# wolfbox/snappy

Hardware: AMD Instinct MI355X
Metric: GiB/s hashed (whole node), bit-exact hashes.yaml, 10k x 1 MiB tree (higher is better)
Workload: dtype u64; 1 GPU; C2: ONE on-disk tree (tmpfs) of 10001 files (10 000 x 1 MiB + the 1 MiB archive stand-in) -> hashes.yaml, sharded over 1 rank(s) on 1 distinct GPU(s); bytes=10486808576, kernel=sha512_split_kernel<true>, tree_home=/dev/shm

## Files before the change

snappy_amd/csrc/hostfill.cpp:

```cpp
#include "hostfill.h"

#include <new>

#include <ctype.h>
#include <dirent.h>
#include <errno.h>
#include <sched.h>
#include <stdio.h>
#include <string.h>
#include <sys/syscall.h>
#include <unistd.h>

#include <algorithm>
#include <atomic>

#if defined(__x86_64__)
#include <immintrin.h>
#endif

namespace snaphash {

namespace {

bool read_small_file(const std::string& path, std::string& out)
{
    FILE* f = fopen(path.c_str(), "r");
    if (!f) return false;
    char buf[4096];
    out.clear();
    size_t r;
    while ((r = fread(buf, 1, sizeof buf, f)) > 0) out.append(buf, r);
    fclose(f);
    return true;
}

constexpr int kMpolDefault = 0, kMpolPreferred = 1;
constexpr unsigned kMpolFNode = 1u << 0, kMpolFAddr = 1u << 1;

}

std::vector<int> parse_cpulist(const std::string& text)
{
    std::vector<int> out;
    const char* p = text.c_str();
    while (*p) {
        while (*p && !isdigit((unsigned char)*p)) ++p;
        if (!*p) break;
        char* end = nullptr;
        const long a = strtol(p, &end, 10);
        long b = a;
        p = end;
        if (*p == '-') { b = strtol(p + 1, &end, 10); p = end; }
        if (a < 0 || b < a || b - a > 65536) break;
        for (long c = a; c <= b; ++c) out.push_back((int)c);
    }
    return out;
}

int numa_node_of_pci(const std::string& sysfs_root, const std::string& bdf_in)
{
    std::string bdf = bdf_in;
    for (char& c : bdf) c = (char)tolower((unsigned char)c);
    if (bdf.empty()) return -1;
    std::string text;
    if (!read_small_file(sysfs_root + "/bus/pci/devices/" + bdf + "/numa_node", text)) return -1;
    char* end = nullptr;
    const long v = strtol(text.c_str(), &end, 10);
    if (end == text.c_str()) return -1;
    return v < 0 ? -1 : (int)v;
}

std::vector<int> numa_cpus_of_node(const std::string& sysfs_root, int node)
{
    std::string text;
    if (node < 0 || !read_small_file(sysfs_root + "/devices/system/node/node" + std::to_string(node) + "/cpulist", text)) return {};
    return parse_cpulist(text);
}

std::vector<int> slice_cpus(const std::vector<int>& all, size_t pos, size_t m)
{
    if (m < 2 || pos >= m) return all;
    std::vector<int> mine;
    for (size_t a = 0; a < all.size();) {
        size_t b = a + 1;
        while (b < all.size() && all[b] == all[b - 1] + 1) ++b;
        const size_t len = b - a;
        for (size_t i = a + len * pos / m; i < a + len * (pos + 1) / m; ++i) mine.push_back(all[i]);
        a = b;
    }
    return mine;
}

int numa_node_count(const std::string& sysfs_root)
{
    int n = 0;
    if (DIR* d = opendir((sysfs_root + "/devices/system/node").c_str())) {
        while (struct dirent* de = readdir(d))
            if (!strncmp(de->d_name, "node", 4) && isdigit((unsigned char)de->d_name[4])) ++n;
        closedir(d);
    }
    return n;
}

bool numa_prefer_node(int node, SavedMemPolicy* saved)
{
#if defined(SYS_set_mempolicy) && defined(SYS_get_mempolicy)
    if (node < 0 || node >= 1024) return false;
    saved->valid = syscall(SYS_get_mempolicy, &saved->mode, saved->mask, (unsigned long)1024 + 1, nullptr, 0ul) == 0;
    unsigned long mask[1024 / (8 * sizeof(unsigned long))] = {0};
    mask[(size_t)node / (8 * sizeof(unsigned long))] |= 1ul << ((size_t)node % (8 * sizeof(unsigned long)));
    return syscall(SYS_set_mempolicy, kMpolPreferred, mask, (unsigned long)1024 + 1) == 0;
#else
    (void)node; (void)saved;
    return false;
#endif
}

void numa_restore_policy(const SavedMemPolicy& saved)
{
#if defined(SYS_set_mempolicy)
    if (saved.valid && saved.mode != kMpolDefault &&
        syscall(SYS_set_mempolicy, saved.mode, saved.mask, (unsigned long)1024 + 1) == 0)
        return;
    (void)syscall(SYS_set_mempolicy, kMpolDefault, nullptr, 0ul);
#else
    (void)saved;
#endif
}

int numa_node_of_address(const void* addr)
{
#if defined(SYS_get_mempolicy)
    int node = -1;
    if (syscall(SYS_get_mempolicy, &node, nullptr, 0ul, addr, (unsigned long)(kMpolFNode | kMpolFAddr)) != 0) return -1;
    return node;
#else
    (void)addr;
    return -1;
#endif
}

unsigned cgroup_cpu_quota(const std::string& sysfs_cgroup_root, const std::string& proc_self_cgroup)
{
    std::string text;
    if (!read_small_file(proc_self_cgroup, text)) return 0;
    double best = 0;
    auto take = [&](double quota, double period) {
        if (quota > 0 && period > 0) { const double c = quota / period; if (best == 0 || c < best) best = c; }
    };
    size_t pos = 0;
    while (pos < text.size()) {
        size_t eol = text.find('\n', pos);
        if (eol == std::string::npos) eol = text.size();
        const std::string line = text.substr(pos, eol - pos);
        pos = eol + 1;
        const size_t c1 = line.find(':'), c2 = c1 == std::string::npos ? c1 : line.find(':', c1 + 1);
        if (c2 == std::string::npos) continue;
        const std::string ctrl = line.substr(c1 + 1, c2 - c1 - 1);
        std::string path = line.substr(c2 + 1);
        const bool v2 = ctrl.empty();
        if (!v2) {
            bool has_cpu = false;
            for (size_t a = 0; a <= ctrl.size();) {
                size_t b = ctrl.find(',', a);
                if (b == std::string::npos) b = ctrl.size();
                if (ctrl.compare(a, b - a, "cpu") == 0) has_cpu = true;
                a = b + 1;
            }
            if (!has_cpu) continue;
        }
        const std::string base = sysfs_cgroup_root + (v2 ? "" : "/" + ctrl);
        for (;;) {
            std::string v;
            if (v2) {
                if (read_small_file(base + path + "/cpu.max", v) && v.compare(0, 3, "max") != 0) {
                    char* end = nullptr;
                    const double q = strtod(v.c_str(), &end);
                    const double per = end ? strtod(end, nullptr) : 0;
                    take(q, per);
                }
            } else {
                std::string pv;
                if (read_small_file(base + path + "/cpu.cfs_quota_us", v) && read_small_file(base + path + "/cpu.cfs_period_us", pv))
                    take(strtod(v.c_str(), nullptr), strtod(pv.c_str(), nullptr));
            }
            if (path.empty() || path == "/") break;
            const size_t slash = path.rfind('/');
            path = slash == 0 || slash == std::string::npos ? "/" : path.substr(0, slash);
        }
    }
    if (best <= 0) return 0;
    return (unsigned)std::max(1.0, best + 0.5);
}

unsigned usable_cpus()
{
    unsigned n = 0;
    cpu_set_t set;
    CPU_ZERO(&set);
    if (sched_getaffinity(0, sizeof set, &set) == 0) {
        const int c = CPU_COUNT(&set);
        if (c > 0) n = (unsigned)c;
    }
    if (n == 0) n = std::max(1u, std::thread::hardware_concurrency());
    static const unsigned quota = cgroup_cpu_quota("/sys/fs/cgroup", "/proc/self/cgroup");
    if (quota && quota < n) n = quota;
    return n;
}


FillPool::~FillPool() { stop(); }

void FillPool::stop()
{
    {
        std::lock_guard<std::mutex> lk(mu_);
        quit_ = true;
    }
    cv_work_.notify_all();
    for (auto& t : th_) if (t.joinable()) t.join();
    th_.clear();
    quit_ = false;
}

void FillPool::configure(unsigned max_threads, const std::vector<int>& cpus)
{
    stop();
    max_threads_ = max_threads;
    cpus_ = cpus;
}

void FillPool::worker(unsigned id)
{
    if (!cpus_.empty()) {
        cpu_set_t set, allowed;
        CPU_ZERO(&set);
        CPU_ZERO(&allowed);
        const bool have_allowed = sched_getaffinity(0, sizeof allowed, &allowed) == 0;
        for (int c : cpus_)
            if (c >= 0 && c < CPU_SETSIZE && (!have_allowed || CPU_ISSET(c, &allowed))) CPU_SET(c, &set);
        if (CPU_COUNT(&set) > 0) (void)sched_setaffinity(0, sizeof set, &set);
    }
    uint64_t seen = 0;
    for (;;) {
        const std::function<void(size_t)>* fn;
        size_t n;
        std::atomic<size_t>* next;
        {
            std::unique_lock<std::mutex> lk(mu_);
            cv_work_.wait(lk, [&] { return quit_ || (epoch_ != seen && id < want_); });
            if (quit_) return;
            seen = epoch_;
            fn = fn_; n = n_; next = next_;
        }
        try {
            for (;;) {
                const size_t i = next->fetch_add(1);
                if (i >= n) break;
                (*fn)(i);
            }
        } catch (...) {
            fn_threw_.store(true);
        }
        {
            std::lock_guard<std::mutex> lk(mu_);
            if (--running_ == 0) cv_done_.notify_all();
        }
    }
}

void FillPool::parallel_for(size_t n, unsigned threads, const std::function<void(size_t)>& fn)
{
    if (n == 0) return;
    unsigned helpers = threads > 1 ? std::min(threads - 1, max_threads_) : 0u;
    if (helpers > n - 1) helpers = (unsigned)(n - 1);
    std::atomic<size_t> next{0};
    if (helpers) {
        std::lock_guard<std::mutex> lk(mu_);
        try {
            while (th_.size() < helpers) { const unsigned id = (unsigned)th_.size(); th_.emplace_back(&FillPool::worker, this, id); }
        } catch (...) {
            helpers = (unsigned)th_.size();
        }
        if (helpers) {
            fn_ = &fn; n_ = n; next_ = &next;
            want_ = helpers;
            running_ = helpers;
            ++epoch_;
        }
    }
    if (helpers) cv_work_.notify_all();
    bool threw = false;
    try {
        for (;;) {
            const size_t i = next.fetch_add(1);
            if (i >= n) break;
            fn(i);
        }
    } catch (...) {
        threw = true;
        next.store(n);
    }
    if (helpers) {
        std::unique_lock<std::mutex> lk(mu_);
        cv_done_.wait(lk, [&] { return running_ == 0; });
        want_ = 0;
        fn_ = nullptr; next_ = nullptr;
    }
    if (fn_threw_.exchange(false) || threw) throw std::bad_alloc();
}


void run_on_threads(unsigned T, const std::function<void(unsigned)>& fn)
{
    if (T <= 1) { fn(0); return; }
    static std::mutex mu;
    static FillPool* pool = [] {
        FillPool* p = new FillPool();
        p->configure(64, {});
        return p;
    }();
    static const pid_t born_in = getpid();
    if (T <= 65 && getpid() == born_in && mu.try_lock()) {
        std::lock_guard<std::mutex> lk(mu, std::adopt_lock);
        pool->parallel_for(T, T, [&fn](size_t t) { fn((unsigned)t); });
        return;
    }
    ThreadJoiner th;
    for (unsigned t = 1; t < T; ++t) th.spawn(fn, t);
    fn(0);
    th.join_all();
}


#if defined(__x86_64__)
namespace {
__attribute__((target("avx2"))) void copy_nt_avx2(uint8_t* dst, const uint8_t* src, size_t n)
{
    const size_t head = (64 - ((uintptr_t)dst & 63)) & 63;
    if (head) { memcpy(dst, src, head); dst += head; src += head; n -= head; }
    size_t lines = n / 64;
    while (lines--) {
        const __m256i a = _mm256_loadu_si256((const __m256i*)src);
        const __m256i b = _mm256_loadu_si256((const __m256i*)(src + 32));
        _mm256_stream_si256((__m256i*)dst, a);
        _mm256_stream_si256((__m256i*)(dst + 32), b);
        src += 64; dst += 64;
    }
    n &= 63;
    if (n) memcpy(dst, src, n);
    _mm_sfence();
}
const bool g_have_avx2 = __builtin_cpu_supports("avx2");
}
#endif

void copy_to_staging(void* dst, const void* src, size_t n)
{
#if defined(__x86_64__)
    if (n >= (32u << 10) && g_have_avx2) { copy_nt_avx2((uint8_t*)dst, (const uint8_t*)src, n); return; }
#endif
    memcpy(dst, src, n);
}

}
```

snappy_amd/csrc/hostfill.h:

```cpp
#pragma once
#include <stddef.h>
#include <stdint.h>

#include <atomic>
#include <condition_variable>
#include <functional>
#include <mutex>
#include <new>
#include <string>
#include <thread>
#include <vector>

namespace snaphash {

int numa_node_of_pci(const std::string& sysfs_root, const std::string& bdf);
std::vector<int> numa_cpus_of_node(const std::string& sysfs_root, int node);
std::vector<int> parse_cpulist(const std::string& text);
int numa_node_count(const std::string& sysfs_root);
std::vector<int> slice_cpus(const std::vector<int>& all, size_t pos, size_t m);

struct SavedMemPolicy {
    bool valid = false;
    int mode = 0;
    unsigned long mask[1024 / (8 * sizeof(unsigned long)) + 1] = {0};
};
bool numa_prefer_node(int node, SavedMemPolicy* saved);
void numa_restore_policy(const SavedMemPolicy& saved);
int numa_node_of_address(const void* addr);
unsigned usable_cpus();
unsigned cgroup_cpu_quota(const std::string& sysfs_cgroup_root, const std::string& proc_self_cgroup);

struct ThreadJoiner {
    std::vector<std::thread> th;
    std::atomic<bool> worker_threw{false};
    ThreadJoiner() = default;
    ThreadJoiner(const ThreadJoiner&) = delete;
    ThreadJoiner& operator=(const ThreadJoiner&) = delete;
    ~ThreadJoiner() { join_quietly(); }
    template <class F, class... A> void spawn(F&& f, A&&... a)
    {
        th.emplace_back([this](auto fn, auto... args) {
            try { fn(args...); } catch (...) { worker_threw.store(true); }
        }, std::forward<F>(f), std::forward<A>(a)...);
    }
    void join_quietly()
    {
        for (auto& t : th)
            if (t.joinable()) t.join();
    }
    void join_all()
    {
        join_quietly();
        if (worker_threw.exchange(false)) throw std::bad_alloc();
    }
};

class FillPool {
public:
    FillPool() = default;
    ~FillPool();
    FillPool(const FillPool&) = delete;
    FillPool& operator=(const FillPool&) = delete;
    void configure(unsigned max_threads, const std::vector<int>& cpus);
    void parallel_for(size_t n, unsigned threads, const std::function<void(size_t)>& fn);
    unsigned max_threads() const { return max_threads_; }
    const std::vector<int>& cpus() const { return cpus_; }

private:
    void worker(unsigned id);
    void stop();
    unsigned max_threads_ = 0;
    std::vector<int> cpus_;
    std::vector<std::thread> th_;
    std::mutex mu_;
    std::condition_variable cv_work_, cv_done_;
    uint64_t epoch_ = 0;
    unsigned want_ = 0;
    unsigned running_ = 0;
    bool quit_ = false;
    const std::function<void(size_t)>* fn_ = nullptr;
    std::atomic<bool> fn_threw_{false};
    size_t n_ = 0;
    std::atomic<size_t>* next_ = nullptr;
};

void run_on_threads(unsigned T, const std::function<void(unsigned)>& fn);

void copy_to_staging(void* dst, const void* src, size_t n);

}
```

snappy_amd/csrc/snaphash_api.cpp:

```cpp
#include <dirent.h>
#include <errno.h>
#include <fcntl.h>
#include <hip/hip_runtime.h>
#include <string.h>
#include <sys/resource.h>
#include <sys/stat.h>
#include <time.h>
#include <unistd.h>

#include <algorithm>
#include <atomic>
#include <queue>
#include <chrono>
#include <string>
#include <thread>
#include <unordered_map>
#include <vector>

#include <dlfcn.h>
#include <rccl/rccl.h>

#include <condition_variable>
#include <functional>
#include <future>
#include <memory>
#include <mutex>

#include "batchplan.h"
#include "engine_bufs.h"
#include "gpu_handles.h"
#include "hostfill.h"
#include "hostpass.h"
#include "hostsha.h"
#include "inflate_host.h"
#include "member_hashers.h"
#include "planner.h"
#include "sha512_core.h"
#include "sha512_kernels.h"
#include "snap_core.h"
#include "tarpack.h"
#include "walk.h"

using namespace snaphash;

namespace {

constexpr uint64_t kDefaultStaging = 256ull << 20;

double now_ms()
{
    using namespace std::chrono;
    return duration<double, std::milli>(steady_clock::now().time_since_epoch()).count();
}

}

struct snaphash_ctx;

struct DevCtx {
    int device = 0;
    int index = 0;
    Stream stream;
    Stream copy_stream;
    uint64_t staging = kDefaultStaging;
    uint32_t kernel_pref = SNAPHASH_KERNEL_AUTO;
    uint32_t deflate_depth = 0;
    uint32_t n_xcd = 8;

    std::vector<SubSlot> sub;
    Slot slot[3];
    HashBufs hash;
    Twin<CmpChunk> cmp;
    DeflateBufs z;
    Stream z_stream;
    Stream z2_stream;
    std::vector<Event> z_ev;
    std::vector<Event> z_part_ev;
    InflateBufs inf;
    Bzip2Bufs bz;
    CrcBufs crc;
    Sha256Bufs sha256;
    BcjBufs bcj;
    Event bcj_ev[2];
    hipStream_t bcj_busy = nullptr;
    XzBufs xz;
    XzEncBufs xe;
    BzEncBufs be;
    Stream f_stream;
    uint64_t fout_gen = 0;

    EventLedger ledger;
    bool pending = false;

    std::string pci_bus_id;
    int numa_node = -1;
    int staging_node = -1;
    int64_t fd_budget = 0;
    int64_t fd_call_budget = -1;
    unsigned fill_cap = 12;
    unsigned fill_call_cap = 0;
    snaphash_ctx* owner = nullptr;
    unsigned owner_cpus_per_engine = 0;
    uint64_t staged_calls = 0;
    double fill_thread_s = 0;
    uint64_t fill_bytes = 0;
    FillPool pool;

    snaphash_stats stats{};
    double t_call0 = 0;
    std::string last_error;

    template <class F> void each_buf(F&& f)
    {
        for (Slot& s : slot) s.each(f);
        for (SubSlot& q : sub) q.jobs.each(f);
        hash.each(f);
        cmp.each(f);
        z.each(f);
        inf.each(f);
        bz.each(f);
        crc.each(f);
        sha256.each(f);
        bcj.each(f);
        xz.each(f);
        xe.each(f);
        be.each(f);
    }
};

namespace {
struct Rccl {
    void* lib = nullptr;
    bool tried = false, ok = false;
    std::string why;
    ncclResult_t (*CommInitAll)(ncclComm_t*, int, const int*) = nullptr;
    ncclResult_t (*CommDestroy)(ncclComm_t) = nullptr;
    ncclResult_t (*AllGather)(const void*, void*, size_t, ncclDataType_t, ncclComm_t, hipStream_t) = nullptr;
    ncclResult_t (*GroupStart)() = nullptr;
    ncclResult_t (*GroupEnd)() = nullptr;
    const char* (*GetErrorString)(ncclResult_t) = nullptr;
    std::vector<ncclComm_t> comms;
};
}

struct snaphash_batch;

struct snaphash_ctx {
    std::vector<std::unique_ptr<DevCtx>> dev;
    uint32_t host_threads = 0;
    bool gpu_only = false;
    unsigned cpus = 1;
    unsigned cpus_call = 0;
    double host_rate = 1.4e9;
    PlanCalib calib;
    std::mutex calib_mu;
    uint32_t flags = 0;
    Rccl rccl;
    std::vector<DevBuf<uint8_t>> d_gather;
    snaphash_stats stats{};
    snaphash_stats_ex ex{};
    snaphash_targz_stats targz{};
    snaphash_unpack_stats unpack{};
    snaphash_xz_check_stats xz_check{};
    snaphash_xz_selfcheck_stats xz_selfcheck{};
    snaphash_xz_filter_stats xz_filter{};
    bool unxz_bcj = false;
    snaphash_bz2_selfcheck_stats bz2_selfcheck{};
    snaphash_block_scan_stats block_scan{};
    std::string last_error;
    snaphash_batch* open_batch = nullptr;
    DevCtx* d0() const { return dev[0].get(); }
};

namespace {

int fail(DevCtx* c, int code, const std::string& msg)
{
    if (c) c->last_error = msg;
    return code;
}
int fail(snaphash_ctx* x, int code, const std::string& msg)
{
// ... 81 lines not shown
    else (void)hipHostFree(p);
}

namespace {

int ensure_slots(DevCtx* c, int nslots = 2, uint64_t want = 0)
{
    if (want == 0 || want > c->staging) want = c->staging;
    for (int k = 0; k < nslots; ++k) {
        Slot& s = c->slot[k];
        HIP_TRY(c, s.ensure(want, c->numa_node));
        if (c->staging_node < 0) { s.h_buf[0] = 0; c->staging_node = numa_node_of_address(s.h_buf.data()); }
        HIP_TRY(c, s.done.ensure(hipEventDisableTiming));
        HIP_TRY(c, s.copied.ensure(hipEventDisableTiming));
    }
    HIP_TRY(c, c->copy_stream.ensure(hipStreamNonBlocking));
    return SNAPHASH_OK;
}

constexpr size_t kSplitMaxStreams = 32768;
constexpr uint64_t kSplitMinBlocks = 32;

uint64_t job_blocks(const Job& j) { return (j.nbytes >> 7) + 1; }

hipError_t launch_kernel(uint32_t k, const Job* d_jobs, size_t n, DevCtx* c, uint8_t* d_digests, bool staged)
{
    if (k == SNAPHASH_KERNEL_QUAD) return launch_quad(d_jobs, (uint32_t)n, c->hash.d_state.data(), d_digests, c->stream);
    if (k == SNAPHASH_KERNEL_PAIR) return launch_pair(d_jobs, (uint32_t)n, c->hash.d_state.data(), d_digests, c->stream, staged);
    if (k == SNAPHASH_KERNEL_SPLIT) return launch_split(d_jobs, (uint32_t)n, c->hash.d_state.data(), d_digests, c->stream);
    return launch_wide(d_jobs, (uint32_t)n, c->hash.d_state.data(), d_digests, c->stream);
}

size_t plan_kernels(const DevCtx* c, const Job* h_jobs, size_t n, uint32_t* k_head, uint32_t* k_tail)
{
    *k_tail = SNAPHASH_KERNEL_WIDE;
    if (c->kernel_pref == SNAPHASH_KERNEL_WIDE || c->kernel_pref == SNAPHASH_KERNEL_SPLIT ||
        c->kernel_pref == SNAPHASH_KERNEL_PAIR || c->kernel_pref == SNAPHASH_KERNEL_QUAD) {
        *k_head = c->kernel_pref;
        return n;
    }
    *k_head = SNAPHASH_KERNEL_PAIR;
    uint64_t blocks = 0;
    for (size_t i = 0; i < n; ++i) blocks += job_blocks(h_jobs[i]);
    if (n <= kSplitMaxStreams) {
        if (blocks >= kSplitMinBlocks * n) return n;
        *k_head = SNAPHASH_KERNEL_WIDE;
        return n;
    }
    if (job_blocks(h_jobs[0]) >= 8 * job_blocks(h_jobs[kSplitMaxStreams - 1]) &&
        job_blocks(h_jobs[0]) >= kSplitMinBlocks) {
        size_t head = 0;
        while (head < kSplitMaxStreams && job_blocks(h_jobs[head]) >= kSplitMinBlocks) ++head;
        return head;
    }
    *k_head = SNAPHASH_KERNEL_WIDE;
    return n;
}

int launch_jobs(DevCtx* c, Job* h_jobs, Job* d_jobs, size_t n, uint8_t* d_digests, hipEvent_t copied = nullptr)
{
    if (n == 0) return SNAPHASH_OK;
    std::stable_sort(h_jobs, h_jobs + n, [](const Job& a, const Job& b) { return a.nbytes > b.nbytes; });
    if (copied) {
        HIP_TRY(c, hipMemcpyAsync(d_jobs, h_jobs, n * sizeof(Job), hipMemcpyHostToDevice, c->copy_stream));
        HIP_TRY(c, hipEventRecord(copied, c->copy_stream));
        HIP_TRY(c, hipStreamWaitEvent(c->stream, copied, 0));
    } else {
        HIP_TRY(c, hipMemcpyAsync(d_jobs, h_jobs, n * sizeof(Job), hipMemcpyHostToDevice, c->stream));
    }
    uint32_t k_head, k_tail;
    const size_t head = plan_kernels(c, h_jobs, n, &k_head, &k_tail);
    Span ev;
    if (int rc = span_begin(c, Ev::Hash, c->stream, &ev)) return rc;
    const bool staged = copied != nullptr;
    hipError_t e = launch_kernel(k_head, d_jobs, head, c, d_digests, staged);
    if (e == hipSuccess && head < n) e = launch_kernel(k_tail, d_jobs + head, n - head, c, d_digests, staged);
    if (e != hipSuccess) return fail(c, SNAPHASH_EDEVICE, std::string("kernel launch: ") + hipGetErrorString(e));
    if (int rc = span_end(c, ev, c->stream)) return rc;
    c->stats.launches += (head < n) ? 2 : 1;
    c->stats.kernel_used = k_head;
    c->pending = true;
    return SNAPHASH_OK;
}

int sync_ctx(DevCtx* c)
{
    if (!c->pending && c->ledger.used() == 0) return SNAPHASH_OK;
    if (c->copy_stream) HIP_TRY(c, hipStreamSynchronize(c->copy_stream));
    HIP_TRY(c, hipStreamSynchronize(c->stream));
    collect_events(c);
    c->pending = false;
    if (c->t_call0 > 0) { c->stats.wall_ms = now_ms() - c->t_call0; c->t_call0 = 0; }
    return SNAPHASH_OK;
}

void begin_call(DevCtx* c)
{
    c->stats = snaphash_stats{};
    c->t_call0 = now_ms();
    c->last_error.clear();
}


struct FdCache {
    std::vector<int> fd;
    std::atomic<int64_t> held{0};
    int64_t budget = 0;
    explicit FdCache(size_t n, int64_t b) : fd(n, -1), budget(b) {}
    ~FdCache() { for (int f : fd) if (f >= 0) close(f); }
    FdCache(const FdCache&) = delete;
    FdCache& operator=(const FdCache&) = delete;
};

int do_read_op(const Source& s, const ReadOp& op, FdCache* cache = nullptr)
{
    if (s.mem) { copy_to_staging(op.dst, s.mem + op.off, op.n); return 0; }
    int err = 0;
    int fd = cache ? cache->fd[op.src] : -1;
    bool cached = fd >= 0;
    if (fd < 0) {
        for (unsigned tries = 0;; ++tries) {
            fd = open(s.path, O_RDONLY | O_CLOEXEC);
            if (fd >= 0 || (errno != EMFILE && errno != ENFILE) || tries >= 2000) break;
            usleep(tries < 100 ? 200 : 2000);
        }
        if (fd < 0) err = errno;
        else if (cache && !op.to_eof && cache->held.load(std::memory_order_relaxed) < cache->budget) {
            cache->fd[op.src] = fd;
            cache->held.fetch_add(1, std::memory_order_relaxed);
            cached = true;
        }
    }
    uint64_t got = 0;
    while (!err && got < op.n) {
        ssize_t r = pread(fd, op.dst + got, op.n - got, (off_t)(op.off + got));
        if (r < 0) { if (errno == EINTR) continue; err = errno; }
        else if (r == 0) err = EIO;
        else got += (uint64_t)r;
    }
    if (!err && op.to_eof) {
        uint8_t probe;
        ssize_t r;
        do r = pread(fd, &probe, 1, (off_t)(op.off + op.n)); while (r < 0 && errno == EINTR);
        if (r > 0) err = EIO;
        else if (r < 0) err = errno;
    }
    if (fd >= 0 && (!cached || op.to_eof || err)) {
        close(fd);
        if (cached) { cache->fd[op.src] = -1; cache->held.fetch_sub(1, std::memory_order_relaxed); }
    }
    return err;
}

void run_reads(DevCtx* c, const std::vector<Source>& src, const std::vector<ReadOp>& ops, std::atomic<int>& first_err,
               std::atomic<int64_t>& first_err_src, FdCache* cache = nullptr, bool alone = false)
{
    static const int forced = [] {
        const char* e = getenv("SNAPHASH_COPY_THREADS");
        const int v = e ? atoi(e) : 0;
        return (v >= 1 && v <= 256) ? v : 0;
    }();
    const bool from_memory = !ops.empty() && src[ops[0].src].mem != nullptr;
    unsigned cap = forced ? (unsigned)forced : std::min(c->fill_cap, from_memory ? 6u : 12u);
    if (!forced && c->fill_call_cap) cap = std::min(cap, c->fill_call_cap);
    if (!forced && alone && !c->fill_call_cap && c->owner) cap = std::max(cap, std::min(c->fill_cap * 2u, c->owner_cpus_per_engine));
    const unsigned T = (unsigned)std::min<size_t>(cap, std::max<size_t>(1, ops.size() / 4));
    const double t_fill0 = now_ms();
    struct FillAccount {
        DevCtx* c; const std::vector<ReadOp>& ops; unsigned T; double t0;
        ~FillAccount()
        {
            uint64_t b = 0;
            for (const ReadOp& op : ops) b += op.n;
            c->fill_bytes += b;
            c->fill_thread_s += (now_ms() - t0) * 1e-3 * T;
        }
    } account{c, ops, T, t_fill0};
    c->pool.parallel_for(ops.size(), T, [&](size_t i) {
        if (first_err.load(std::memory_order_relaxed)) return;
        const ReadOp& op = ops[i];
        const int err = do_read_op(src[op.src], op, cache);
        if (err) {
            int z = 0;
            if (first_err.compare_exchange_strong(z, err)) first_err_src.store(op.src);
        }
    });
}

struct EngineSpans { float gpu = 0, copy_busy = 0, copy = 0; };
EngineSpans engine_spans(DevCtx* c)
{
    EngineSpans sp;
    if (c->copy_stream) (void)hipStreamSynchronize(c->copy_stream);
    (void)hipStreamSynchronize(c->stream);
    Span first_copy, last_copy, last_kernel, first;
    c->ledger.each([&](Ev kind, const Span& s) {
        if (!first.a) first = s;
        if (kind == Ev::H2d) {
            if (!first_copy.a) first_copy = s;
            last_copy = s;
            sp.copy_busy += span_ms(s);
        } else if (kind == Ev::Hash) last_kernel = s;
    });
    if (first_copy.a) {
        (void)hipEventElapsedTime(&sp.gpu, first_copy.a, (last_kernel.b ? last_kernel : first).b);
        (void)hipEventElapsedTime(&sp.copy, first_copy.a, last_copy.b);
    }
    return sp;
}

int hash_sources(DevCtx* c, const std::vector<Source>& src, uint8_t* digests, uint64_t* states, int* err_no,
                 int64_t* err_src)
{
    const size_t n = src.size();
    if (err_no) *err_no = 0;
    if (err_src) *err_src = -1;
    if (n == 0) return SNAPHASH_OK;
    HIP_TRY(c, hipSetDevice(c->device));
    uint64_t job_bytes = 0;
    bool empty_files = false;
    for (const Source& sc : src) { job_bytes += sc.gpu_len; empty_files |= sc.len == 0 && sc.path != nullptr; }
    const bool from_memory = src[0].mem != nullptr;
    const uint64_t slot_caps[3] = {c->slot[0].cap(), c->slot[1].cap(), c->slot[2].cap()};
    const BatchGeometry g = batch_geometry(job_bytes, n, c->staging, slot_caps, from_memory);
    int rc = ensure_slots(c, (int)g.nslots, g.slot_bytes);
    if (rc) return rc;
    HIP_TRY(c, c->hash.ensure(n, true));
    if (c->sub.size() < g.nsub) c->sub.resize(g.nsub);
    for (unsigned q = 0; q < g.nsub; ++q) {
        SubSlot& ss = c->sub[q];
        HIP_TRY(c, ss.done.ensure(hipEventDisableTiming));
        HIP_TRY(c, ss.copied.ensure(hipEventDisableTiming));
        ss.busy = false;
    }

    c->fill_thread_s = 0;
    c->fill_bytes = 0;
    BatchPlanner plan(src.data(), n, job_bytes, g.S_full, BatchKnobs::from_env());
    std::atomic<int> first_err{0};
    std::atomic<int64_t> first_err_src{-1};
    std::vector<ReadOp> ops;
    FdCache fds(from_memory ? 0 : n, c->fd_call_budget >= 0 ? std::min(c->fd_call_budget, c->fd_budget) : c->fd_budget);
    double t_wait = 0, t_plan = 0, t_read = 0, t_launch = 0;
    const double t_engine0 = now_ms();
    double t_first_copy = 0;
    size_t n_copies = 0;

    while (!plan.active.empty()) {
        const unsigned batch = plan.batch, q = batch % g.nsub;
        SubSlot& sl = c->sub[q];
        uint8_t* const sl_h = c->slot[q / g.per_slot].h_buf.data() + (uint64_t)(q % g.per_slot) * g.S_full;
        uint8_t* const sl_d = c->slot[q / g.per_slot].d_buf.data() + (uint64_t)(q % g.per_slot) * g.S_full;
        const double tb0 = now_ms();
        if (sl.busy) { HIP_TRY(c, hipEventSynchronize(sl.done)); sl.busy = false; }
        const double tb1 = now_ms();
        t_wait += tb1 - tb0;
        HIP_TRY(c, sl.jobs.ensure(plan.active.size()));
        const Batch b = plan.next(sl.jobs.h.data(), ops, (uint64_t)(uintptr_t)sl_h, (uint64_t)(uintptr_t)sl_d);
        c->stats.blocks += b.blocks;
        static const bool trace_batches = getenv("SNAPHASH_TRACE_BATCHES") != nullptr;
        if (trace_batches) trace_batch(stderr, c->index, batch, b, sl.jobs.h.data(), (uint64_t)(uintptr_t)sl_d, plan.active.size());
        if (empty_files)
            for (size_t k = 0; k < b.nj; ++k) {
                const Job& j = sl.jobs.h[k];
                if (j.nbytes == 0 && src[j.idx].len == 0 && src[j.idx].path) ops.push_back(ReadOp{j.idx, 0, 0, sl_h, true});
            }
        const double tb2 = now_ms();
        t_plan += tb2 - tb1;

        run_reads(c, src, ops, first_err, first_err_src, from_memory ? nullptr : &fds, batch == 0);
        if (first_err.load()) break;
        const double tb3 = now_ms();
        t_read += tb3 - tb2;
        if (trace_batches)
            fprintf(stderr, "snaphash engine %d: batch %u: at %.2f ms: waited %.2f, planned %.2f, filled %.2f ms (%zu streams begun, %.1f GB/s)\n", c->index, batch,
                    tb0 - t_engine0, tb1 - tb0, tb2 - tb1, tb3 - tb2, b.n_new, (double)b.used / ((tb3 - tb2) * 1e6 + 1e-9));

        if (b.used) {
            if (batch == 0) t_first_copy = now_ms() - t_engine0;
            ++n_copies;
            Span ev;
            if ((rc = span_begin(c, Ev::H2d, c->copy_stream, &ev))) return rc;
            HIP_TRY(c, hipMemcpyAsync(sl_d, sl_h, b.used, hipMemcpyHostToDevice, c->copy_stream));
            if ((rc = span_end(c, ev, c->copy_stream))) return rc;
        }
        rc = launch_jobs(c, sl.jobs.h.data(), sl.jobs.d.data(), b.nj, c->hash.d_digests.data(), sl.copied);
        if (rc) return rc;
        HIP_TRY(c, hipEventRecord(sl.done, c->stream));
        sl.busy = true;
        t_launch += now_ms() - tb3;
    }

    const double ts0 = now_ms();
    static const bool trace_tree = getenv("SNAPHASH_TRACE_TREE") != nullptr;
    const EngineSpans sp = trace_tree && c->ledger.used() > 1 ? engine_spans(c) : EngineSpans{};
    rc = sync_ctx(c);
    if (trace_tree)
        fprintf(stderr, "snaphash engine %d: %u batches; waiting for a slot %.1f ms, planning %.1f ms, reads %.1f ms, enqueue %.1f ms, drain %.1f ms; "
                        "first copy enqueued at %.2f ms, copies busy %.2f of %.2f ms, first copy -> last kernel %.2f ms, engine %.2f ms\n",
                c->index, plan.batch, t_wait, t_plan, t_read, t_launch, now_ms() - ts0, t_first_copy, sp.copy_busy, sp.copy, sp.gpu, now_ms() - t_engine0);
    for (SubSlot& ss : c->sub) ss.busy = false;
    if (rc) return rc;
    if (first_err.load()) {
        const int64_t s = first_err_src.load();
        if (err_no) *err_no = first_err.load();
        if (err_src) *err_src = s;
        return fail(c, SNAPHASH_EIO,
                    std::string(s >= 0 && src[s].path ? src[s].path : "<buffer>") + ": " + strerror(first_err.load()));
    }
    if (digests) HIP_TRY(c, hipMemcpy(digests, c->hash.d_digests.data(), n * 64, hipMemcpyDeviceToHost));
    if (states) HIP_TRY(c, hipMemcpy(states, c->hash.d_state.data(), n * 64, hipMemcpyDeviceToHost));
    for (size_t i = 0; i < n; ++i) c->stats.bytes_hashed += src[i].gpu_len;
    c->stats.streams = n;
    if (c->owner) {
        std::lock_guard<std::mutex> lk(c->owner->calib_mu);
        const double planned = c->owner->ex.planned_gpu_ms, took = now_ms() - t_engine0;
        const bool take_fill = c->staged_calls++ > 0 && !(planned > 0 && took > 3.0 * planned);
        c->owner->calib.observe_call(!from_memory, (double)c->fill_bytes, (double)n, (double)n_copies, c->stats.h2d_ms * 1e-3, c->fill_thread_s, take_fill);
    }
    return SNAPHASH_OK;
}


bool rccl_load(snaphash_ctx* x)
{
    Rccl& r = x->rccl;
    if (r.tried) return r.ok;
    r.tried = true;
    for (const char* name : {"librccl.so.1", "librccl.so", "/opt/rocm/lib/librccl.so.1"}) {
        r.lib = dlopen(name, RTLD_NOW | RTLD_LOCAL);
        if (r.lib) break;
    }
    if (!r.lib) { r.why = "librccl.so not found"; return false; }
    r.CommInitAll = (decltype(r.CommInitAll))dlsym(r.lib, "ncclCommInitAll");
    r.CommDestroy = (decltype(r.CommDestroy))dlsym(r.lib, "ncclCommDestroy");
    r.AllGather = (decltype(r.AllGather))dlsym(r.lib, "ncclAllGather");
    r.GroupStart = (decltype(r.GroupStart))dlsym(r.lib, "ncclGroupStart");
    r.GroupEnd = (decltype(r.GroupEnd))dlsym(r.lib, "ncclGroupEnd");
    r.GetErrorString = (decltype(r.GetErrorString))dlsym(r.lib, "ncclGetErrorString");
    if (!r.CommInitAll || !r.CommDestroy || !r.AllGather || !r.GroupStart || !r.GroupEnd) {
        r.why = "librccl.so lacks a required symbol";
        return false;
    }
    std::vector<int> devs;
    for (auto& d : x->dev) devs.push_back(d->device);
    std::vector<int> uniq = devs;
    std::sort(uniq.begin(), uniq.end());
    if (std::adjacent_find(uniq.begin(), uniq.end()) != uniq.end()) {
        r.why = "a device ordinal repeats in the ctx (RCCL needs one rank per GPU)";
        return false;
    }
    r.comms.assign(devs.size(), nullptr);
    const ncclResult_t e = r.CommInitAll(r.comms.data(), (int)devs.size(), devs.data());
    if (e != ncclSuccess) {
        r.why = std::string("ncclCommInitAll: ") + (r.GetErrorString ? r.GetErrorString(e) : "error");
        r.comms.clear();
        return false;
    }
    r.ok = true;
    return true;
}

int gather_digest_slabs(snaphash_ctx* x, const std::vector<size_t>& cnt, size_t kmax, std::vector<uint8_t>& rows)
{
    const size_t nd = x->dev.size();
    rows.assign(nd * kmax * 64, 0);
    const double t0 = now_ms();
    bool use_rccl = !(x->flags & SNAPHASH_FLAG_NO_RCCL) && rccl_load(x);
    if (use_rccl) {
        x->d_gather.resize(nd);
        for (size_t d = 0; d < nd; ++d) {
            DevCtx* c = x->dev[d].get();
            HIP_TRY(c, hipSetDevice(c->device));
            if (x->d_gather[d].reserve(nd * kmax * 64) != hipSuccess)
                return fail(x, SNAPHASH_ENOMEM, "hipMalloc of the gather buffer failed");
            HIP_TRY(x, c->hash.ensure(kmax, true));
        }
        Rccl& r = x->rccl;
        ncclResult_t e = r.GroupStart();
        for (size_t d = 0; d < nd && e == ncclSuccess; ++d) {
            DevCtx* c = x->dev[d].get();
            (void)hipSetDevice(c->device);
            e = r.AllGather(c->hash.d_digests.data(), x->d_gather[d].data(), kmax * 64, ncclUint8, r.comms[d], c->stream);
        }
        const ncclResult_t e2 = r.GroupEnd();
        if (e == ncclSuccess) e = e2;
        if (e != ncclSuccess) {
            r.ok = false;
            r.why = std::string("RCCL all-gather: ") + (r.GetErrorString ? r.GetErrorString(e) : "error");
            use_rccl = false;
        }
    }
    if (use_rccl) {
        Rccl& r = x->rccl;
        (void)r;
        for (size_t d = 0; d < nd; ++d) {
            DevCtx* c = x->dev[d].get();
            HIP_TRY(c, hipSetDevice(c->device));
            HIP_TRY(c, hipStreamSynchronize(c->stream));
        }
        DevCtx* c0 = x->d0();
        HIP_TRY(c0, hipSetDevice(c0->device));
        HIP_TRY(c0, hipMemcpy(rows.data(), x->d_gather[0].data(), nd * kmax * 64, hipMemcpyDeviceToHost));
        x->ex.gather_kind = 1;
        if (x->flags & SNAPHASH_FLAG_CHECK_GATHER) {
            std::vector<uint8_t> own(kmax * 64);
            for (size_t d = 0; d < nd; ++d) {
                DevCtx* c = x->dev[d].get();
                HIP_TRY(c, hipSetDevice(c->device));
                if (cnt[d]) HIP_TRY(c, hipMemcpy(own.data(), c->hash.d_digests.data(), cnt[d] * 64, hipMemcpyDeviceToHost));
                if (memcmp(own.data(), rows.data() + d * kmax * 64, cnt[d] * 64) != 0)
                    return fail(x, SNAPHASH_EDEVICE, "RCCL-gathered digest slab differs from the device's own copy");
            }
            x->ex.gather_checked = 1;
        }
    } else {
        for (size_t d = 0; d < nd; ++d) {
            DevCtx* c = x->dev[d].get();
            HIP_TRY(c, hipSetDevice(c->device));
            if (cnt[d]) HIP_TRY(c, hipMemcpy(rows.data() + d * kmax * 64, c->hash.d_digests.data(), cnt[d] * 64, hipMemcpyDeviceToHost));
        }
        x->ex.gather_kind = 2;
    }
    x->ex.gather_ms = now_ms() - t0;
    return SNAPHASH_OK;
}


double measure_host_rate()
{
    static std::mutex mu;
    static double smoothed = 0;
    std::vector<uint8_t> buf(512u << 10, 0x5a);
    HostSha hs;
    uint8_t out[64];
    double rate[5];
    int n = 0;
    for (int rep = 0; rep < 5; ++rep) {
        host_sha512_init(hs);
        const double t0 = now_ms();
        host_sha512_update(hs, buf.data(), buf.size());
        host_sha512_final(hs, out);
        const double dt = (now_ms() - t0) * 1e-3;
        if (dt > 0) rate[n++] = (double)buf.size() / dt;
    }
    if (n == 0) return 0.40e9;
    std::sort(rate, rate + n);
    const double median = rate[n / 2];
    if (!(median > 50e6)) return 0.40e9;
    std::lock_guard<std::mutex> lk(mu);
    smoothed = smoothed > 0 ? 0.75 * smoothed + 0.25 * median : median;
    return smoothed;
}
// ... 2233 lines not shown
```

Before: 49.99 GiB/s.

## Plan next batch while pool threads fill the current one

```diff
diff --git a/snappy_amd/csrc/engine_pipeline.h b/snappy_amd/csrc/engine_pipeline.h
--- /dev/null
+++ b/snappy_amd/csrc/engine_pipeline.h
@@ -0,0 +1,35 @@
+#pragma once
+
+namespace snaphash {
+
+template <class Hooks>
+int run_engine_pipeline(Hooks& h, unsigned nsub, bool ahead)
+{
+    if (!h.more()) return 0;
+    if (int rc = h.wait_slot(0u)) return rc;
+    if (int rc = h.plan(0u)) return rc;
+    h.begin_fill(0u);
+    for (unsigned k = 0;; ++k) {
+        bool next_planned = false;
+        if (ahead && nsub > 1 && h.more() && h.slot_free_now(k + 1)) {
+            if (int rc = h.plan(k + 1)) { (void)h.finish_fill(k); return rc; }
+            next_planned = true;
+        }
+        if (!h.finish_fill(k)) {
+            if (next_planned) h.dropped(k + 1);
+            return 0;
+        }
+        if (next_planned) h.begin_fill(k + 1);
+        if (int rc = h.enqueue(k)) {
+            if (next_planned) (void)h.finish_fill(k + 1);
+            return rc;
+        }
+        if (next_planned) continue;
+        if (!h.more()) return 0;
+        if (int rc = h.wait_slot(k + 1)) return rc;
+        if (int rc = h.plan(k + 1)) return rc;
+        h.begin_fill(k + 1);
+    }
+}
+
+}
diff --git a/snappy_amd/csrc/hostfill.cpp b/snappy_amd/csrc/hostfill.cpp
--- a/snappy_amd/csrc/hostfill.cpp
+++ b/snappy_amd/csrc/hostfill.cpp
@@ -2,6 +2,7 @@
 
 #include <new>
 
+#include <assert.h>
 #include <ctype.h>
 #include <dirent.h>
 #include <errno.h>
@@ -243,24 +244,23 @@
     }
     uint64_t seen = 0;
     for (;;) {
-        const std::function<void(size_t)>* fn;
         size_t n;
-        std::atomic<size_t>* next;
         {
             std::unique_lock<std::mutex> lk(mu_);
             cv_work_.wait(lk, [&] { return quit_ || (epoch_ != seen && id < want_); });
             if (quit_) return;
             seen = epoch_;
-            fn = fn_; n = n_; next = next_;
+            n = n_;
         }
         try {
             for (;;) {
-                const size_t i = next->fetch_add(1);
+                const size_t i = next_.fetch_add(1);
                 if (i >= n) break;
-                (*fn)(i);
+                fn_(i);
             }
         } catch (...) {
             fn_threw_.store(true);
+            next_.store(n);
         }
         {
             std::lock_guard<std::mutex> lk(mu_);
@@ -269,13 +269,18 @@
     }
 }
 
-void FillPool::parallel_for(size_t n, unsigned threads, const std::function<void(size_t)>& fn)
-{
-    if (n == 0) return;
-    unsigned helpers = threads > 1 ? std::min(threads - 1, max_threads_) : 0u;
-    if (helpers > n - 1) helpers = (unsigned)(n - 1);
-    std::atomic<size_t> next{0};
-    if (helpers) {
+void FillPool::begin(size_t n, unsigned threads, std::function<void(size_t)> fn)
+{
+    assert(!open_ && "FillPool::begin: the job before this one was not finished");
+    open_ = true;
+    unsigned helpers = (n > 0 && threads > 1) ? std::min(threads - 1, max_threads_) : 0u;
+    if (helpers > n - 1 && n > 0) helpers = (unsigned)(n - 1);
+    fn_ = std::move(fn);
+    n_ = n;
+    next_.store(0);
+    helpers_ = 0;
+    if (!helpers) return;
+    {
         std::lock_guard<std::mutex> lk(mu_);
         try {
             while (th_.size() < helpers) { const unsigned id = (unsigned)th_.size(); th_.emplace_back(&FillPool::worker, this, id); }
@@ -283,30 +288,38 @@
             helpers = (unsigned)th_.size();
         }
         if (helpers) {
-            fn_ = &fn; n_ = n; next_ = &next;
             want_ = helpers;
             running_ = helpers;
             ++epoch_;
         }
+        helpers_ = helpers;
     }
     if (helpers) cv_work_.notify_all();
+}
+
+void FillPool::finish()
+{
+    assert(open_ && "FillPool::finish without begin");
     bool threw = false;
+    const size_t n = n_;
     try {
         for (;;) {
-            const size_t i = next.fetch_add(1);
+            const size_t i = next_.fetch_add(1);
             if (i >= n) break;
-            fn(i);
+            fn_(i);
         }
     } catch (...) {
         threw = true;
-        next.store(n);
-    }
-    if (helpers) {
+        next_.store(n);
+    }
+    if (helpers_) {
         std::unique_lock<std::mutex> lk(mu_);
         cv_done_.wait(lk, [&] { return running_ == 0; });
         want_ = 0;
-        fn_ = nullptr; next_ = nullptr;
-    }
+    }
+    helpers_ = 0;
+    fn_ = nullptr;
+    open_ = false;
     if (fn_threw_.exchange(false) || threw) throw std::bad_alloc();
 }
 
diff --git a/snappy_amd/csrc/hostfill.h b/snappy_amd/csrc/hostfill.h
--- a/snappy_amd/csrc/hostfill.h
+++ b/snappy_amd/csrc/hostfill.h
@@ -62,7 +62,9 @@
     FillPool(const FillPool&) = delete;
     FillPool& operator=(const FillPool&) = delete;
     void configure(unsigned max_threads, const std::vector<int>& cpus);
-    void parallel_for(size_t n, unsigned threads, const std::function<void(size_t)>& fn);
+    void parallel_for(size_t n, unsigned threads, const std::function<void(size_t)>& fn) { begin(n, threads, fn); finish(); }
+    void begin(size_t n, unsigned threads, std::function<void(size_t)> fn);
+    void finish();
     unsigned max_threads() const { return max_threads_; }
     const std::vector<int>& cpus() const { return cpus_; }
 
@@ -78,10 +80,12 @@
     unsigned want_ = 0;
     unsigned running_ = 0;
     bool quit_ = false;
-    const std::function<void(size_t)>* fn_ = nullptr;
+    std::function<void(size_t)> fn_;
     std::atomic<bool> fn_threw_{false};
     size_t n_ = 0;
-    std::atomic<size_t>* next_ = nullptr;
+    std::atomic<size_t> next_{0};
+    unsigned helpers_ = 0;
+    bool open_ = false;
 };
 
 void run_on_threads(unsigned T, const std::function<void(unsigned)>& fn);
diff --git a/snappy_amd/csrc/snaphash_api.cpp b/snappy_amd/csrc/snaphash_api.cpp
--- a/snappy_amd/csrc/snaphash_api.cpp
+++ b/snappy_amd/csrc/snaphash_api.cpp
@@ -28,6 +28,7 @@
 
 #include "batchplan.h"
 #include "engine_bufs.h"
+#include "engine_pipeline.h"
 #include "gpu_handles.h"
 #include "hostfill.h"
 #include "hostpass.h"
@@ -415,8 +416,9 @@
     return err;
 }
 
-void run_reads(DevCtx* c, const std::vector<Source>& src, const std::vector<ReadOp>& ops, std::atomic<int>& first_err,
-               std::atomic<int64_t>& first_err_src, FdCache* cache = nullptr, bool alone = false)
+struct FillRun { const std::vector<ReadOp>* ops = nullptr; unsigned T = 0; double t0 = 0; };
+FillRun begin_reads(DevCtx* c, const std::vector<Source>& src, const std::vector<ReadOp>& ops, std::atomic<int>& first_err,
+                    std::atomic<int64_t>& first_err_src, FdCache* cache = nullptr, unsigned wide = 0)
 {
     static const int forced = [] {
         const char* e = getenv("SNAPHASH_COPY_THREADS");
@@ -426,20 +428,10 @@
     const bool from_memory = !ops.empty() && src[ops[0].src].mem != nullptr;
     unsigned cap = forced ? (unsigned)forced : std::min(c->fill_cap, from_memory ? 6u : 12u);
     if (!forced && c->fill_call_cap) cap = std::min(cap, c->fill_call_cap);
-    if (!forced && alone && !c->fill_call_cap && c->owner) cap = std::max(cap, std::min(c->fill_cap * 2u, c->owner_cpus_per_engine));
+    if (!forced && wide && !c->fill_call_cap && c->owner) cap = std::max(cap, std::min(std::min(c->fill_cap * 2u, c->owner_cpus_per_engine), wide));
     const unsigned T = (unsigned)std::min<size_t>(cap, std::max<size_t>(1, ops.size() / 4));
-    const double t_fill0 = now_ms();
-    struct FillAccount {
-        DevCtx* c; const std::vector<ReadOp>& ops; unsigned T; double t0;
-        ~FillAccount()
-        {
-            uint64_t b = 0;
-            for (const ReadOp& op : ops) b += op.n;
-            c->fill_bytes += b;
-            c->fill_thread_s += (now_ms() - t0) * 1e-3 * T;
-        }
-    } account{c, ops, T, t_fill0};
-    c->pool.parallel_for(ops.size(), T, [&](size_t i) {
+    const FillRun run{&ops, T, now_ms()};
+    c->pool.begin(ops.size(), T, [&src, &ops, &first_err, &first_err_src, cache](size_t i) {
         if (first_err.load(std::memory_order_relaxed)) return;
         const ReadOp& op = ops[i];
         const int err = do_read_op(src[op.src], op, cache);
@@ -448,6 +440,29 @@
             if (first_err.compare_exchange_strong(z, err)) first_err_src.store(op.src);
         }
     });
+    return run;
+}
+
+void finish_reads(DevCtx* c, const FillRun& run)
+{
+    struct FillAccount {
+        DevCtx* c; const FillRun& run;
+        ~FillAccount()
+        {
+            uint64_t b = 0;
+            for (const ReadOp& op : *run.ops) b += op.n;
+            c->fill_bytes += b;
+            c->fill_thread_s += (now_ms() - run.t0) * 1e-3 * run.T;
+        }
+    } account{c, run};
+    c->pool.finish();
+}
+
+void run_reads(DevCtx* c, const std::vector<Source>& src, const std::vector<ReadOp>& ops, std::atomic<int>& first_err,
+               std::atomic<int64_t>& first_err_src, FdCache* cache = nullptr, unsigned wide = 0)
+{
+    const FillRun run = begin_reads(c, src, ops, first_err, first_err_src, cache, wide);
+    finish_reads(c, run);
 }
 
 struct EngineSpans { float gpu = 0, copy_busy = 0, copy = 0; };
@@ -471,6 +486,129 @@
     }
     return sp;
 }
+
+struct EngineLoop {
+    DevCtx* const c;
+    const std::vector<Source>& src;
+    const BatchGeometry g;
+    const bool empty_files, from_memory;
+    BatchPlanner planner;
+    std::atomic<int> first_err{0};
+    std::atomic<int64_t> first_err_src{-1};
+    FdCache fds;
+    struct Staged {
+        Batch b;
+        std::vector<ReadOp> ops;
+        unsigned q = 0;
+        uint8_t *sl_h = nullptr, *sl_d = nullptr;
+        double waited = 0, planned = 0;
+        double t_fill0 = 0;
+        FillRun run;
+    } st[2];
+    bool filling = false;
+    double t_wait = 0, t_plan = 0, t_read = 0, t_launch = 0;
+    const double t_engine0 = now_ms();
+    double t_first_copy = 0;
+    size_t n_copies = 0;
+    unsigned n_ahead = 0;
+    const bool trace_batches = getenv("SNAPHASH_TRACE_BATCHES") != nullptr;
+    const bool wide_new = [] { const char* e = getenv("SNAPHASH_FILL_WIDE_NEW"); return !(e && e[0] == '0'); }();
+
+    EngineLoop(DevCtx* c_, const std::vector<Source>& src_, const BatchGeometry& g_, uint64_t job_bytes, bool empty_files_, bool from_memory_)
+        : c(c_), src(src_), g(g_), empty_files(empty_files_), from_memory(from_memory_),
+          planner(src_.data(), src_.size(), job_bytes, g_.S_full, BatchKnobs::from_env()),
+          fds(from_memory_ ? 0 : src_.size(), c_->fd_call_budget >= 0 ? std::min(c_->fd_call_budget, c_->fd_budget) : c_->fd_budget) {}
+    ~EngineLoop()
+    {
+        if (filling) { try { c->pool.finish(); } catch (...) {} }
+    }
+    EngineLoop(const EngineLoop&) = delete;
+    EngineLoop& operator=(const EngineLoop&) = delete;
+
+    SubSlot& sub(unsigned k) { return c->sub[k % g.nsub]; }
+    bool more() const { return !planner.active.empty(); }
+    bool slot_free_now(unsigned k)
+    {
+        SubSlot& sl = sub(k);
+        if (!sl.busy) return true;
+        if (hipEventQuery(sl.done) == hipSuccess) { sl.busy = false; return true; }
+        (void)hipGetLastError();
+        return false;
+    }
+    int wait_slot(unsigned k)
+    {
+        SubSlot& sl = sub(k);
+        const double t0 = now_ms();
+        if (sl.busy) { HIP_TRY(c, hipEventSynchronize(sl.done)); sl.busy = false; }
+        st[k & 1].waited = now_ms() - t0;
+        t_wait += st[k & 1].waited;
+        return SNAPHASH_OK;
+    }
+    int plan_batch(unsigned k, bool ahead)
+    {
+        Staged& s = st[k & 1];
+        SubSlot& sl = sub(k);
+        const double t0 = now_ms();
+        if (ahead) { s.waited = 0; ++n_ahead; }
+        s.q = k % g.nsub;
+        s.sl_h = c->slot[s.q / g.per_slot].h_buf.data() + (uint64_t)(s.q % g.per_slot) * g.S_full;
+        s.sl_d = c->slot[s.q / g.per_slot].d_buf.data() + (uint64_t)(s.q % g.per_slot) * g.S_full;
+        HIP_TRY(c, sl.jobs.ensure(planner.active.size()));
+        s.b = planner.next(sl.jobs.h.data(), s.ops, (uint64_t)(uintptr_t)s.sl_h, (uint64_t)(uintptr_t)s.sl_d);
+        c->stats.blocks += s.b.blocks;
+        if (trace_batches) trace_batch(stderr, c->index, k, s.b, sl.jobs.h.data(), (uint64_t)(uintptr_t)s.sl_d, planner.active.size());
+        if (empty_files)
+            for (size_t i = 0; i < s.b.nj; ++i) {
+                const Job& j = sl.jobs.h[i];
+                if (j.nbytes == 0 && src[j.idx].len == 0 && src[j.idx].path) s.ops.push_back(ReadOp{j.idx, 0, 0, s.sl_h, true});
+            }
+        s.planned = now_ms() - t0;
+        t_plan += s.planned;
+        return SNAPHASH_OK;
+    }
+    int plan(unsigned k) { return plan_batch(k, filling); }
+    void begin_fill(unsigned k)
+    {
+        Staged& s = st[k & 1];
+        s.t_fill0 = now_ms();
+        const unsigned wide = k == 0 ? UINT_MAX : (wide_new && s.b.n_new > 0) ? 16u : 0u;
+        s.run = begin_reads(c, src, s.ops, first_err, first_err_src, from_memory ? nullptr : &fds, wide);
+        filling = true;
+    }
+    bool finish_fill(unsigned k)
+    {
+        Staged& s = st[k & 1];
+        filling = false;
+        finish_reads(c, s.run);
+        if (first_err.load()) return false;
+        const double filled = now_ms() - s.t_fill0;
+        t_read += filled;
+        if (trace_batches)
+            fprintf(stderr, "snaphash engine %d: batch %u: at %.2f ms: waited %.2f, planned %.2f, filled %.2f ms (%zu streams begun, %.1f GB/s)\n", c->index, k,
+                    s.t_fill0 - t_engine0, s.waited, s.planned, filled, s.b.n_new, (double)s.b.used / (filled * 1e6 + 1e-9));
+        return true;
+    }
+    int enqueue(unsigned k)
+    {
+        Staged& s = st[k & 1];
+        SubSlot& sl = sub(k);
+        const double t0 = now_ms();
+        if (s.b.used) {
+            if (k == 0) t_first_copy = now_ms() - t_engine0;
+            ++n_copies;
+            Span ev;
+            if (int rc = span_begin(c, Ev::H2d, c->copy_stream, &ev)) return rc;
+            HIP_TRY(c, hipMemcpyAsync(s.sl_d, s.sl_h, s.b.used, hipMemcpyHostToDevice, c->copy_stream));
+            if (int rc = span_end(c, ev, c->copy_stream)) return rc;
+        }
+        if (int rc = launch_jobs(c, sl.jobs.h.data(), sl.jobs.d.data(), s.b.nj, c->hash.d_digests.data(), sl.copied)) return rc;
+        HIP_TRY(c, hipEventRecord(sl.done, c->stream));
+        sl.busy = true;
+        t_launch += now_ms() - t0;
+        return SNAPHASH_OK;
+    }
+    void dropped(unsigned) {}
+};
 
 int hash_sources(DevCtx* c, const std::vector<Source>& src, uint8_t* digests, uint64_t* states, int* err_no,
                  int64_t* err_src)
@@ -499,60 +637,15 @@
 
     c->fill_thread_s = 0;
     c->fill_bytes = 0;
-    BatchPlanner plan(src.data(), n, job_bytes, g.S_full, BatchKnobs::from_env());
-    std::atomic<int> first_err{0};
-    std::atomic<int64_t> first_err_src{-1};
-    std::vector<ReadOp> ops;
-    FdCache fds(from_memory ? 0 : n, c->fd_call_budget >= 0 ? std::min(c->fd_call_budget, c->fd_budget) : c->fd_budget);
-    double t_wait = 0, t_plan = 0, t_read = 0, t_launch = 0;
-    const double t_engine0 = now_ms();
-    double t_first_copy = 0;
-    size_t n_copies = 0;
-
-    while (!plan.active.empty()) {
-        const unsigned batch = plan.batch, q = batch % g.nsub;
-        SubSlot& sl = c->sub[q];
-        uint8_t* const sl_h = c->slot[q / g.per_slot].h_buf.data() + (uint64_t)(q % g.per_slot) * g.S_full;
-        uint8_t* const sl_d = c->slot[q / g.per_slot].d_buf.data() + (uint64_t)(q % g.per_slot) * g.S_full;
-        const double tb0 = now_ms();
-        if (sl.busy) { HIP_TRY(c, hipEventSynchronize(sl.done)); sl.busy = false; }
-        const double tb1 = now_ms();
-        t_wait += tb1 - tb0;
-        HIP_TRY(c, sl.jobs.ensure(plan.active.size()));
-        const Batch b = plan.next(sl.jobs.h.data(), ops, (uint64_t)(uintptr_t)sl_h, (uint64_t)(uintptr_t)sl_d);
-        c->stats.blocks += b.blocks;
-        static const bool trace_batches = getenv("SNAPHASH_TRACE_BATCHES") != nullptr;
-        if (trace_batches) trace_batch(stderr, c->index, batch, b, sl.jobs.h.data(), (uint64_t)(uintptr_t)sl_d, plan.active.size());
-        if (empty_files)
-            for (size_t k = 0; k < b.nj; ++k) {
-                const Job& j = sl.jobs.h[k];
-                if (j.nbytes == 0 && src[j.idx].len == 0 && src[j.idx].path) ops.push_back(ReadOp{j.idx, 0, 0, sl_h, true});
-            }
-        const double tb2 = now_ms();
-        t_plan += tb2 - tb1;
-
-        run_reads(c, src, ops, first_err, first_err_src, from_memory ? nullptr : &fds, batch == 0);
-        if (first_err.load()) break;
-        const double tb3 = now_ms();
-        t_read += tb3 - tb2;
-        if (trace_batches)
-            fprintf(stderr, "snaphash engine %d: batch %u: at %.2f ms: waited %.2f, planned %.2f, filled %.2f ms (%zu streams begun, %.1f GB/s)\n", c->index, batch,
-                    tb0 - t_engine0, tb1 - tb0, tb2 - tb1, tb3 - tb2, b.n_new, (double)b.used / ((tb3 - tb2) * 1e6 + 1e-9));
-
-        if (b.used) {
-            if (batch == 0) t_first_copy = now_ms() - t_engine0;
-            ++n_copies;
-            Span ev;
-            if ((rc = span_begin(c, Ev::H2d, c->copy_stream, &ev))) return rc;
-            HIP_TRY(c, hipMemcpyAsync(sl_d, sl_h, b.used, hipMemcpyHostToDevice, c->copy_stream));
-            if ((rc = span_end(c, ev, c->copy_stream))) return rc;
-        }
-        rc = launch_jobs(c, sl.jobs.h.data(), sl.jobs.d.data(), b.nj, c->hash.d_digests.data(), sl.copied);
-        if (rc) return rc;
-        HIP_TRY(c, hipEventRecord(sl.done, c->stream));
-        sl.busy = true;
-        t_launch += now_ms() - tb3;
-    }
+    const char* const pipe_env = getenv("SNAPHASH_ENGINE_PIPELINE");
+    const bool plan_ahead = !(pipe_env && pipe_env[0] == '0');
+    EngineLoop loop(c, src, g, job_bytes, empty_files, from_memory);
+    rc = run_engine_pipeline(loop, g.nsub, plan_ahead);
+    if (rc) return rc;
+    const std::atomic<int>& first_err = loop.first_err;
+    const std::atomic<int64_t>& first_err_src = loop.first_err_src;
+    const double t_engine0 = loop.t_engine0;
+    const size_t n_copies = loop.n_copies;
 
     const double ts0 = now_ms();
     static const bool trace_tree = getenv("SNAPHASH_TRACE_TREE") != nullptr;
@@ -560,8 +653,9 @@
     rc = sync_ctx(c);
     if (trace_tree)
         fprintf(stderr, "snaphash engine %d: %u batches; waiting for a slot %.1f ms, planning %.1f ms, reads %.1f ms, enqueue %.1f ms, drain %.1f ms; "
-                        "first copy enqueued at %.2f ms, copies busy %.2f of %.2f ms, first copy -> last kernel %.2f ms, engine %.2f ms\n",
-                c->index, plan.batch, t_wait, t_plan, t_read, t_launch, now_ms() - ts0, t_first_copy, sp.copy_busy, sp.copy, sp.gpu, now_ms() - t_engine0);
+                        "first copy enqueued at %.2f ms, copies busy %.2f of %.2f ms, first copy -> last kernel %.2f ms, engine %.2f ms; %u batches planned ahead\n",
+                c->index, loop.planner.batch, loop.t_wait, loop.t_plan, loop.t_read, loop.t_launch, now_ms() - ts0, loop.t_first_copy, sp.copy_busy, sp.copy, sp.gpu,
+                now_ms() - t_engine0, loop.n_ahead);
     for (SubSlot& ss : c->sub) ss.busy = false;
     if (rc) return rc;
     if (first_err.load()) {
```

Result: no change. 50.02 GiB/s, median of 3 (+0.1%).
